# zoltanmaric/h264-fer

Measured on AMD Instinct MI355X. Metric: macroblocks/sec encode (1080p full-search ME) + bit-exact bitstream vs ref, higher is better.
Workload: dtype u8; 1 GPU; 1080p IPPP encode, full-search +-16 ME (BASELINE configs[2]); content=textured, coded_size=1920x1072, streams_per_gpu=256, contexts_per_gpu=1, gop=30, qp=12, window=32, maxdiff=3, parallelism=1 x 256 independent closed-GOP streams

## Files before the change

### h264-fer_amd/__init__.py

```python
from .ferhip import (FerHip, FerHipError, Decoder, LiveDecoder, access_units, DeviceBuffer, Y4MReader, decode_streams, unescape_nal, lib_path,
                     load_library, mb_unit, cavlc_blocks, mc_sub_mb_parts, MBU_QT, MBU_DEC4, MBU_DEC16, MBU_DECC, MBU_SKIP, TUNE_RESOLVE_WGS, TUNE_RESOLVE_GROUP, TUNE_SPECULATE, TUNE_OVERLAP_SORT, RC_CQP, RC_ABR, RC_QUALITY, QM_SSE, QM_SSIM,
                     QUALITY_RING, Quality, NAL_SLICE, NAL_IDR, NAL_AUTO, NAL_NONE, AU_PARAM_SETS, AU, frame_nal_blocks, frame_nal_blocks_raw,
                     NAL_UNIT, SPLIT_PREFIX, split_nal_blocks, split_nal_blocks_raw, FMT_I420, FMT_NV12, Pic, pic_table,
                     AU_AVCC, IN_ANNEXB, IN_AVCC, split_avcc_blocks_raw)
from .synth import gen_frame, gen_frames, crop_to_mb, pad_to_mb
from .shard import gops_of_rank, merge_gop_streams, split_nals
```

### h264-fer_amd/csrc/fer_internal.h

```cpp
#pragma once
#include "fer_dev.h"
#include "../../include/ferhip.h"

struct FerSortTmp {
    uint4 *rec1;
    uint16_t *keyT;
    uint8_t *dig2;
    uint16_t *skey;
    uint32_t *rec_tmp;
    void *tmp;
    size_t tmp_bytes;
};

size_t fer_sort_tmp_bytes(int n, int S);
void fer_launch_refprep(const FerDev &d, FerSortTmp &t, const int *types, hipStream_t st);
void fer_launch_interp(const FerDev &d, hipStream_t st);
void fer_launch_features(const FerDev &d, hipStream_t st);
void fer_launch_sort(const FerDev &d, FerSortTmp &t, hipStream_t st);
void fer_launch_sort_keys(const FerDev &d, FerSortTmp &t, hipStream_t st);
void fer_launch_sort_radix(const FerDev &d, FerSortTmp &t, hipStream_t st);
void fer_launch_sort_finish(const FerDev &d, FerSortTmp &t, hipStream_t st);
void fer_launch_me_walk(const FerDev &d, hipStream_t st);
void fer_launch_frame_sad(const FerDev &d, const uint8_t *skip, hipStream_t st);
void fer_launch_me_pre(const FerDev &d, hipStream_t st);
void fer_launch_me_spec(const FerDev &d, hipStream_t st);
void fer_launch_me_resolve(const FerDev &d, hipStream_t st);
void fer_launch_basic_stat(const FerDev &d, hipStream_t st);
void fer_launch_p_resid(const FerDev &d, hipStream_t st);
void fer_launch_intra(const FerDev &d, hipStream_t st);
void fer_launch_cavlc(const FerDev &d, hipStream_t st);
void fer_launch_rc_plan(const FerDev &d, hipStream_t st);
int fer_quality_groups(const FerDev &d);
void fer_launch_quality(const FerDev &d, int flags, int slot, hipStream_t st);
void fer_launch_carry_ref(const FerDev &d, hipStream_t st);
void fer_launch_reset_stream(const FerDev &d, int s, int qpw, hipStream_t st);
void fer_launch_decode_parse(const FerDev &d, const DecBatch &B, hipStream_t st);
void fer_launch_decode_recon(const FerDev &dslice, bool anyP, bool anyIntra, hipStream_t st);
void fer_launch_decode_out(const FerDev &d, const uint8_t *set, const int2 *map, int n, uint8_t *dst, hipStream_t st);
void fer_launch_decode_out_win(const FerDev &d, const uint8_t *set, const int2 *map, int n, uint8_t *dst, const int *win, hipStream_t st);
void fer_launch_pad_ingest(const FerDev &d, uint8_t *set, const uint8_t *src, int dw, int dh, const uint8_t *present, hipStream_t st);
void fer_launch_pic_ingest(const FerDev &d, uint8_t *set, const ferhip_pic *d_pics, int format, int dw, int dh, hipStream_t st);
void fer_launch_pic_emit(const FerDev &d, const uint8_t *set, const ferhip_pic *d_pics, int format, const int *win, hipStream_t st);
void fer_launch_pic_emit_slots(const FerDev &d, const uint8_t *set, const int2 *map, int n, uint8_t *dst, int format, uint32_t pitch_y,
                               uint32_t pitch_c, size_t slot_bytes, const int *win, hipStream_t st);
```

### h264-fer_amd/csrc/fer_mbunit.hip

```cpp
#include "fer_cavlc_dev.h"
#include "fer_ctx.h"

__device__ __forceinline__ void mbu_scan(const int c[16], int32_t *list, bool ac)
{
#pragma unroll
    for (int k = ac ? 1 : 0; k < 16; k++) list[ac ? k - 1 : k] = c[c_zz[k]];
    if (ac) list[15] = 0;
}
__device__ __forceinline__ void mbu_invscan(const int32_t *list, int c[16], bool ac, int dc)
{
#pragma unroll
    for (int k = 0; k < 16; k++) c[c_zz[k]] = ac ? (k == 0 ? dc : list[k - 1]) : list[k];
}

__global__ __launch_bounds__(64) void k_mb_unit(const ferhip_mb_job *jobs, ferhip_mb_result *res, int n)
{
    __shared__ int dcl[16], dcc[2][4], dcdeq[2][4], dcy[16];
    const int j = blockIdx.x, lane = threadIdx.x;
    if (j >= n) return;
    const ferhip_mb_job &J = jobs[j];
    ferhip_mb_result &R = res[j];
    const int op = J.op, qp = J.qp, qpc = J.qpc;
    const bool luma = lane < 16, chroma = lane >= 16 && lane < 24;
    const int blk = lane & 15, cpl = (lane - 16) >> 2, cblk = (lane - 16) & 3;
// ... 104 lines not shown
            int dq[16];
            mbu_invscan(J.dc16, cc, false, 0);
            inv_dc_luma(cc, dq, qp);
#pragma unroll
            for (int i = 0; i < 16; i++) dcy[i] = dq[i];
        }
        __syncthreads();
        if (luma) {
            mbu_invscan(J.ac16[blk], cc, true, dcy[(y0 >> 2) * 4 + (x0 >> 2)]);
            inv4x4(cc, r, qp, true);
            store_rec(r);
        }
    } else if (op == FERHIP_MBU_DECC) {
        if (lane == 16 || lane == 20) {
            int q[4], dq[4];
#pragma unroll
            for (int i = 0; i < 4; i++) q[i] = J.cdc[cpl][i];
            inv_dc_chroma(q, dq, qpc);
#pragma unroll
            for (int i = 0; i < 4; i++) dcdeq[cpl][i] = dq[i];
        }
        __syncthreads();
        if (chroma) {
            mbu_invscan(J.cac[cpl][cblk], cc, true, dcdeq[cpl][cblk]);
            inv4x4(cc, r, qpc, true);
            store_rec(r);
        }
    } else if (op == FERHIP_MBU_SKIP) {
#pragma unroll
        for (int i = 0; i < 16; i++) cc[i] = 0;
        inv4x4(cc, r, luma ? qp : qpc, !luma);
        if (luma || chroma) store_rec(r);
    }
}

extern "C" int ferhip_mb_unit(const ferhip_mb_job *jobs, ferhip_mb_result *results, size_t n)
{
    if (!jobs || !results || n == 0) return FERHIP_E_ARG;
    ferhip_mb_job *dj = nullptr;
    ferhip_mb_result *dr = nullptr;
    auto body = [&]() -> int {
        CK(hipMalloc((void **)&dj, n * sizeof *dj));
        CK(hipMalloc((void **)&dr, n * sizeof *dr));
        CK(hipMemcpy(dj, jobs, n * sizeof *dj, hipMemcpyHostToDevice));
        CK(hipMemset(dr, 0, n * sizeof *dr));
        hipLaunchKernelGGL(k_mb_unit, dim3((unsigned)n), dim3(64), 0, 0, dj, dr, (int)n);
        CK(hipGetLastError());
        CK(hipMemcpy(results, dr, n * sizeof *dr, hipMemcpyDeviceToHost));
        return 0;
    };
    const int rc = body();
    hipFree(dj);
    hipFree(dr);
    return rc;
}

__global__ __launch_bounds__(64) void k_cavlc_blocks(const int32_t *coef, const int32_t *nC, const int32_t *maxn, int n, uint32_t *bits,
                                                     uint32_t *nbits, int32_t *tc, uint32_t *nbits_size)
{
    __shared__ int16_t stage[16 * 64];
    const int i = blockIdx.x * 64 + threadIdx.x;
    if (i >= n) return;
    int16_t *st = stage + threadIdx.x;
    const int m = maxn[i];
    unsigned nz = 0;
#pragma unroll
    for (int k = 0; k < 16; k++) {
        const int v = k < m ? coef[(size_t)i * 16 + k] : 0;
        st[k * 64] = (int16_t)v;
        nz |= (v != 0 ? 1u : 0u) << k;
    }
    BitW w;
    bw_init<true>(w, bits + (size_t)i * 16, 16, 0);
    cavlc_block_core<true>(w, nz, m, nC[i], st, 64);
    bw_flush<true>(w);
    nbits[i] = w.bits;
    tc[i] = __popc(nz);
    BitW ws;
    bw_init<false>(ws, nullptr, 0, 0);
    cavlc_block_core<false>(ws, nz, m, nC[i], st, 64);
    nbits_size[i] = ws.bits;
}

extern "C" int ferhip_cavlc_blocks(const int32_t *coef, const int32_t *nC, const int32_t *max_num_coeff, size_t n, uint8_t *bits,
                                   uint32_t *nbits, int32_t *total_coeff)
{
    if (!coef || !nC || !max_num_coeff || !bits || !nbits || !total_coeff || n == 0) return FERHIP_E_ARG;
    int32_t *dc = nullptr, *dn = nullptr, *dm = nullptr, *dt = nullptr;
    uint32_t *db = nullptr, *dl = nullptr, *ds = nullptr;
    std::vector<uint32_t> sz(n);
    auto body = [&]() -> int {
        CK(hipMalloc((void **)&dc, n * 64));
        CK(hipMalloc((void **)&dn, n * 4));
        CK(hipMalloc((void **)&dm, n * 4));
        CK(hipMalloc((void **)&dt, n * 4));
        CK(hipMalloc((void **)&db, n * 64));
        CK(hipMalloc((void **)&dl, n * 4));
        CK(hipMalloc((void **)&ds, n * 4));
        CK(hipMemcpy(dc, coef, n * 64, hipMemcpyHostToDevice));
        CK(hipMemcpy(dn, nC, n * 4, hipMemcpyHostToDevice));
        CK(hipMemcpy(dm, max_num_coeff, n * 4, hipMemcpyHostToDevice));
        CK(hipMemset(db, 0, n * 64));
        hipLaunchKernelGGL(k_cavlc_blocks, dim3((unsigned)((n + 63) / 64)), dim3(64), 0, 0, dc, dn, dm, (int)n, db, dl, dt, ds);
        CK(hipGetLastError());
        CK(hipMemcpy(bits, db, n * 64, hipMemcpyDeviceToHost));
        CK(hipMemcpy(nbits, dl, n * 4, hipMemcpyDeviceToHost));
// ... 166 lines not shown
```

### h264-fer_amd/csrc/fer_me.hip

```cpp
#include <stdlib.h>
#include "fer_internal.h"
#include "fer_mvpred.h"

#define INF_M 1000000000

struct WList {
    int m;
    int xy;
};

__device__ __forceinline__ int pack_xy(int x, int y) { return (x & 0xffff) | (y << 16); }
__device__ __forceinline__ int unp_x(int xy) { return (int)(short)(xy & 0xffff); }
__device__ __forceinline__ int unp_y(int xy) { return xy >> 16; }

__device__ __forceinline__ void wl_insert(WList &L, int K, int lane, bool valid, int m, int xy)
{
    int thr = lane_bcast(L.m, K - 1);
    unsigned long long mask = __ballot(valid && m < thr);
    while (mask) {
        int src = __ffsll((long long)mask) - 1;
        mask &= mask - 1;
        int cm = lane_bcast(m, src), cxy = lane_bcast(xy, src);
        int pos = __popcll(__ballot(lane < K && L.m <= cm));
        if (pos < K) {
            int um = FER_DPP(L.m, DPP_WAVE_SHR1), uxy = FER_DPP(L.xy, DPP_WAVE_SHR1);
            if (lane > pos && lane < K) {
                L.m = um;
                L.xy = uxy;
            } else if (lane == pos) {
                L.m = cm;
                L.xy = cxy;
            }
        }
    }
}

#define WAVE_LDS_SYNC()                                    \
    do {                                                   \
        __builtin_amdgcn_fence(__ATOMIC_SEQ_CST, "wavefront"); \
        __builtin_amdgcn_wave_barrier();                   \
    } while (0)
__device__ __forceinline__ int lds_rank64(const unsigned *p, unsigned mine, int n4 = 16)
{
    const uint4 *q = (const uint4 *)p;
    int r = 0;
#pragma unroll 4
    for (int i = 0; i < n4; i++) {
        uint4 k = q[i];
        r += (int)(k.x < mine) + (int)(k.y < mine) + (int)(k.z < mine) + (int)(k.w < mine);
    }
    return r;
}

template <int NB, bool ORDERED, class RAW, class FIN, class ARR>
__device__ __forceinline__ bool select_topk_ex(const int (&v)[NB], int K, int lane, int *sel, WList &L, RAW raw, FIN fin, ARR arr)
{
    unsigned *A = (unsigned *)sel, *B = A + 64;
    int *Ci = sel + 128, *Di = sel + 192;
    const unsigned long long lt = (1ull << lane) - 1ull;
    int lmin = 0x7fffffff, lmax = -1, total = 0;
#pragma unroll
    for (int u = 0; u < NB; u++) {
        total += __popcll(__ballot(v[u] >= 0));
        lmin = (int)min((unsigned)lmin, (unsigned)v[u]);
        lmax = max(lmax, v[u]);
    }
    const int need = min(K, total);
    L.m = INF_M;
    L.xy = 0;
    if (need == 0) return true;
    int c = 65;
    if (!__any(lmax >= (1 << 26))) {
        B[lane] = 0xffffffffu;
        int T0 = 0x7fffffff;
        if (__popcll(__ballot(lmin != 0x7fffffff)) >= need) {
            int lo = 0, hi = (1 << 21) - 1;
            if (__popcll(__ballot(lmin <= hi)) >= need) {
                while (lo < hi) {
                    const int mid = (lo + hi) >> 1;
                    if (__popcll(__ballot(lmin <= mid)) >= need)
                        hi = mid;
                    else
                        lo = mid + 1;
                }
                T0 = lo;
            } else {
                T0 = 1 << 21;
            }
        }
        WAVE_LDS_SYNC();
        if (T0 < (1 << 21) && NB * 64 <= 2048) {
            int nsurv = 0;
#pragma unroll
            for (int u = 0; u < NB; u++) {
                const bool take = (unsigned)v[u] <= (unsigned)T0;
                const unsigned long long mk = __ballot(take);
                if (mk) {
                    const int slot = nsurv + (int)__builtin_amdgcn_mbcnt_hi((uint32_t)(mk >> 32), __builtin_amdgcn_mbcnt_lo((uint32_t)mk, 0u));
                    if (take && slot < 64) {
                        B[slot] = ((unsigned)v[u] << 11) | (unsigned)arr(u);
                        Ci[slot] = raw(u);
                    }
                    nsurv += __popcll(mk);
                }
            }
            WAVE_LDS_SYNC();
            c = nsurv;
        }
    }
    if (c <= 64) {
        WAVE_LDS_SYNC();
        const unsigned mine = B[lane];
        const int mypay = Ci[lane];
        const int rk = lds_rank64(B, mine, (__builtin_amdgcn_readfirstlane(c) + 3) >> 2);
        WAVE_LDS_SYNC();
        if (lane < c && rk < need) {
            A[rk] = mine >> 11;
            Di[rk] = mypay;
        }
        WAVE_LDS_SYNC();
        if (lane < need) {
            L.m = (int)A[lane];
            L.xy = fin(Di[lane]);
        }
        WAVE_LDS_SYNC();
        return true;
    }
    if (!ORDERED) return false;
    int *key = sel, *kxy = sel + 64, *key2 = sel + 128, *kxy2 = sel + 192;
    int lo = wave_min(lmin), hi;
    if (__popcll(__ballot(lmin != 0x7fffffff)) >= need)
        hi = wave_max(lmin != 0x7fffffff ? lmin : -1);
    else
        hi = wave_max(lmax);
    while (lo < hi) {
        int mid = lo + ((hi - lo) >> 1);
        int cnt = 0;
#pragma unroll
        for (int u = 0; u < NB; u++) cnt += __popcll(__ballot(v[u] >= 0 && v[u] <= mid));
        if (cnt >= need)
            hi = mid;
        else
// ... 332 lines not shown
    su[4] = wave_sum((px & 3) > 1 ? 0 : v);
    if (lane < 5) d.suma[pidx * 5 + lane] = su[lane];
    if (d.basic) {
        if (lane == 0) {
            d.st3n[pidx] = 0;
            d.v0[pidx] = 0;
        }
        return;
    }
    const SuPk sp = su_pack(su);
    PP_MARK(0)

    WList L;
    L.m = INF_M;
    L.xy = 0;
    const int R = window / 2, n = 2 * R + 1;
    const int r2 = window / 16, n2w = 2 * r2 + 1, nloc = n2w * n2w * 16;
    const uint16_t *F0 = d.feat0 + (size_t)s * 6 * ysz;
    const int wb = (n * n + 63) >> 6;
    if ((WIN == 32 || WIN == 16) && !FER_DBGF(d, 3)) {
        constexpr int WCH = 6;
        constexpr int NN = (WIN ? WIN : 32) + 1;
        constexpr int NBc = WIN ? WIN : 32, RPB = 64 / NBc, NWB = (NN + RPB - 1) / RPB;
        constexpr int LB = LocalGeo<RRL>::NB;
        static_assert(LB <= 7, "ME_SEL_NB leaves room for 7 local batches");
        const int ix = lane % NBc, r0 = lane / NBc;
        const int rx = sx - R + ix;
        const bool xok = rx >= 0 && rx < W;
        const int wx = iabs(ix - R) + 4;
        const uint32_t colo = (uint32_t)iclamp(rx, 0, W - 1) * 12u, rowb = (uint32_t)W * 12u;
        auto fin = [&](int idx) {
            if (idx < wb * 64) return pack_xy((idx / n - R) * 4, (idx % n - R) * 4);
            int c = idx - wb * 64;
            int frac = c & 15, pos = c >> 4;
            return pack_xy((pos / n2w - r2) * 4 + (frac & 3), (pos % n2w - r2) * 4 + (frac >> 2));
        };
        uint32_t k0w[NWB];
#pragma unroll
        for (int b2 = 0; b2 < NWB; b2++) {
            const int ry = iclamp(sy - R + b2 * RPB + r0, 0, H - 1);
            k0w[b2] = *(const uint32_t *)((const char *)F0 + (colo + __umul24((uint32_t)ry, rowb)));
        }
        const uint32_t k0c = feat0_load(F0, W, H, sy - R + min(lane, NN - 1), sx + R).a;
        local_metrics<RRL>(ip, W, H, sx - r2, sy - r2, sp, lane, (uint32_t *)wide_m, sel_lds, 0, 2, &ld);
        int vloc[LB];
        unsigned lminl = 0xffffffffu;
#pragma unroll
        for (int u = 0; u < LB; u++) {
            vloc[u] = sel_lds[u * 64 + lane];
            lminl = min(lminl, (unsigned)vloc[u]);
        }
        int T = 0x7fffffff;
        if (__popcll(__ballot(lminl < (1u << 21))) >= 33) {
            int lo = 0, hi = (1 << 21) - 1;
            while (lo < hi) {
                const int mid = (lo + hi) >> 1;
                if (__popcll(__ballot(lminl <= (unsigned)mid)) >= 33)
                    hi = mid;
                else
                    lo = mid + 1;
            }
            T = lo;
        }
        int *surv = wide_m;
        int ns = 0;
        const uint32_t s0 = (uint32_t)su[0];
        bool done = false;
        if (T != 0x7fffffff) {
#pragma unroll
            for (int b2 = 0; b2 < NWB; b2++) {
                const int iy = b2 * RPB + r0;
                const int ry = sy - R + iy;
                const uint32_t lb = __umul24(5u * (uint32_t)(wx + iabs(iy - R)), __builtin_amdgcn_sad_u16(k0w[b2] & 0xffffu, s0, 0u));
                const bool take = xok && ry >= 0 && ry < H && iy < NN && lb <= (uint32_t)T;
                const unsigned long long mk = __ballot(take);
                if (mk) {
                    const int slot = ns + (int)__builtin_amdgcn_mbcnt_hi((uint32_t)(mk >> 32), __builtin_amdgcn_mbcnt_lo((uint32_t)mk, 0u));
                    if (take && slot < 128) surv[slot] = ix * NN + iy;
                    ns += __popcll(mk);
                }
            }
            {
                const int iy = lane, ry = sy - R + iy;
                const uint32_t lb = __umul24(5u * (uint32_t)(R + 4 + iabs(iy - R)), __builtin_amdgcn_sad_u16(k0c & 0xffffu, s0, 0u));
                const bool take = iy < NN && sx + R < W && ry >= 0 && ry < H && lb <= (uint32_t)T;
                const unsigned long long mk = __ballot(take);
                if (mk) {
                    const int slot = ns + (int)__builtin_amdgcn_mbcnt_hi((uint32_t)(mk >> 32), __builtin_amdgcn_mbcnt_lo((uint32_t)mk, 0u));
                    if (take && slot < 128) surv[slot] = (NN - 1) * NN + iy;
                    ns += __popcll(mk);
                }
            }
            WAVE_LDS_SYNC();
            if (ns <= 128) {
                int v[2 + LB], ar[2];
#pragma unroll
                for (int b2 = 0; b2 < 2; b2++) {
                    v[b2] = -1;
                    ar[b2] = 0;
                    if (b2 * 64 < ns) {
                        const int idx = b2 * 64 + lane;
                        const bool on = idx < ns;
                        const int ai = on ? surv[idx] : 0;
                        const int cix = ai / NN, ciy = ai - cix * NN;
                        const FeatRec f = feat0_load(F0, W, H, sy - R + ciy, sx - R + cix);
                        const int m = (int)__umul24((uint32_t)(iabs(cix - R) + iabs(ciy - R) + 4), (uint32_t)feat_dist_w(f.a, f.b, f.c, sp));
                        v[b2] = on ? m : -1;
                        ar[b2] = ai;
                    }
                }
#pragma unroll
                for (int u = 0; u < LB; u++) v[2 + u] = vloc[u];
                WAVE_LDS_SYNC();
                auto arrv = [&](int u) { return u < 2 ? ar[u < 2 ? u : 0] : wb * 64 + (u - 2) * 64 + lane; };
                done = select_topk_ex<2 + LB, false>(v, 33, lane, sel_lds, L, arrv, fin, arrv);
            }
        }
        PP_MARK(1)
#ifdef FER_STATS
        if (lane == 0) {
            atomicAdd((unsigned long long *)&d.timing[48], 1ull);
            atomicAdd((unsigned long long *)&d.timing[49], done ? 0ull : 1ull);
            atomicAdd((unsigned long long *)&d.timing[50], (unsigned long long)ns);
            atomicAdd((unsigned long long *)&d.timing[51], T == 0x7fffffff ? 1ull : 0ull);
            atomicAdd((unsigned long long *)&d.timing[52], (unsigned long long)(T == 0x7fffffff ? 0 : T));
        }
#endif
        if (!done) {
            WAVE_LDS_SYNC();
            auto wide_load = [&](int iy0, FeatRec (&fr)[WCH]) {
#pragma unroll
                for (int q = 0; q < WCH; q++) {
                    int ry = iclamp(sy - R + iy0 + q * RPB + r0, 0, H - 1);
                    const uint32_t *r = (const uint32_t *)((const char *)F0 + (colo + __umul24((uint32_t)ry, rowb)));
                    fr[q].a = r[0];
                    fr[q].b = r[1];
                    fr[q].c = r[2];
                }
            };
            auto wide_eval = [&](int iy0, const FeatRec (&fr)[WCH]) {
#pragma unroll
                for (int q = 0; q < WCH; q++) {
                    const int iy = iy0 + q * RPB + r0;
                    const int ry = sy - R + iy;
                    const int m = (int)__umul24((uint32_t)(wx + iabs(iy - R)), (uint32_t)feat_dist_w(fr[q].a, fr[q].b, fr[q].c, sp));
                    const int bad = (xok && ry >= 0 && ry < H) ? 0 : -1;
                    wide_m[iy < n ? ix * n + iy : ME_WIDE_LDS - 1] = m | bad;
                }
            };
            {
                constexpr int STEP = RPB * WCH;
                FeatRec fa[WCH], fb[WCH];
                wide_load(0, fa);
                for (int iy0 = 0; iy0 < n; iy0 += 2 * STEP) {
                    if (iy0 + STEP < n) wide_load(iy0 + STEP, fb);
                    wide_eval(iy0, fa);
                    if (iy0 + STEP < n) {
                        if (iy0 + 2 * STEP < n) wide_load(iy0 + 2 * STEP, fa);
                        wide_eval(iy0 + STEP, fb);
                    }
                }
            }
            {
                const int iy = min(lane, n - 1);
                const int rxl = sx + R, ry = sy - R + iy;
                FeatRec f = feat0_load(F0, W, H, ry, rxl);
                int m = (R + 4 + iabs(iy - R)) * feat_dist_w(f.a, f.b, f.c, sp);
                if (!(rxl < W && ry >= 0 && ry < H)) m = -1;
                if (lane < n) wide_m[(n - 1) * n + iy] = m;
            }
            __syncthreads();
            int v[ME_SEL_NB];
#pragma unroll
            for (int u = 0; u < ME_SEL_NB; u++) {
                v[u] = -1;
                if (u < wb) {
                    int c = u * 64 + lane;
                    if (c < n * n) v[u] = wide_m[c];
                } else if (u - wb < LB) {
                    v[u] = vloc[u - wb < LB ? u - wb : 0];
                }
            }
            WAVE_LDS_SYNC();
            auto raw = [&](int u) { return u * 64 + lane; };
            PP_MARK(2)
            select_topk<ME_SEL_NB>(v, 33, lane, sel_lds, L, raw, fin);
        }
        PP_MARK(3)
    } else {
        for (int base = 0; base < n * n && !FER_DBGF(d, 1); base += 64) {
            int c = base + lane;
            int tx = c / n - R, ty = c % n - R;
            int rx = sx + tx, ry = sy + ty;
            bool ok = c < n * n && rx >= 0 && rx < W && ry >= 0 && ry < H;
            int m = 0;
            if (ok) m = (iabs(tx) + iabs(ty) + 4) * feat_dist_rec(F0 + ((size_t)ry * W + rx) * 6, sp);
            wl_insert(L, 33, lane, ok, m, pack_xy(tx * 4, ty * 4));
        }
        for (int base = 0; base < nloc && !FER_DBGF(d, 2); base += 64) {
            int c = base + lane;
            int frac = c & 15, pos = c >> 4;
            int tx = pos / n2w - r2, ty = pos % n2w - r2;
            int rx = sx + tx, ry = sy + ty;
            bool ok = c < nloc && rx >= 0 && rx < W && ry >= 0 && ry < H;
            int m = 0;
            if (ok) {
                const FeatRec f = feat_rec_direct(ip, W, H, frac, ry, rx);
                m = (iabs(tx) + iabs(ty) + 4) * feat_dist_w(f.a, f.b, f.c, sp);
            }
            wl_insert(L, 33, lane, ok, m, pack_xy(tx * 4 + (frac & 3), ty * 4 + (frac >> 2)));
        }
    }
    const int n3 = __popcll(__ballot(lane < 33 && L.m < 100000000));
    int v0 = 0;
    if (!FER_DBGF(d, 4)) {
        const SrcBlk SB = src_block_load(Y, W, sx, sy);
        const int cx = unp_x(L.xy), cy = unp_y(L.xy);
        const int sad = sad_lane(ip, W, H, sx, sy, lane < n3 ? cx : 0, lane < n3 ? cy : 0, SB);
        if (lane < n3) {
            int *o = d.st3 + (pidx * 33 + lane) * 3;
            o[0] = cx;
            o[1] = cy;
            o[2] = sad;
        }
        const int wk = wave_min(lane < n3 ? (sad << 6) | lane : 0x7fffffff);
        if (wk != 0x7fffffff) v0 = lane_bcast(L.xy, wk & 63);
    }
    if (lane == 0) {
        d.st3n[pidx] = n3;
        d.v0[pidx] = v0;
    }

}

__device__ __forceinline__ bool wave_mask_bit(unsigned long long m) { return __builtin_amdgcn_inverse_ballot_w64(m); }
__device__ __forceinline__ unsigned long long wave_ballot(bool p) { return __builtin_amdgcn_ballot_w64(p); }
struct NoProbe {
    __device__ __forceinline__ int operator()(int) const { return 0; }
};
template <bool QUIRK, class SINK, class PROBE = NoProbe>
__device__ __forceinline__ int walk_buckets_q(const FerDev &d, int s, const int (&su)[5], const SuPk &sp, int sx, int sy, int lane,
                                              uint32_t *tbl, int halt_cnt, int &jend, SINK sink, uint32_t max_slice = 0xffffffffu,
                                              bool skip0 = false, PROBE probe = PROBE())
{
    int tren = 0;
    jend = 180;
    const int kt = d.kt;
    const uint32_t *kol2 = d.kol2 + (size_t)s * 16384 * kt;
    const uint32_t *srec = d.sort_rec;
    const int n0 = QUIRK ? d.zero_cnt[s] : 0;
    const uint32_t npos = (uint32_t)(d.W * d.H), g0 = (uint32_t)s * npos;
    const uint16_t *F0 = d.feat0 + (size_t)s * 6 * d.ysz;
    const int t_lo = QUIRK ? 0 : (max(sx - 279, 0) >> d.ktw_shift), t_hi = QUIRK ? kt - 1 : (min(sx + 279, d.W - 1) >> d.ktw_shift);
    auto qstart = [&](int a) -> uint32_t {
        if (a <= 0) return g0;
        if (a == 1) return g0 + min(2u * (uint32_t)n0, npos);
        if (a >= 16384) return g0 + npos;
        return kol2[(size_t)a * kt] - (uint32_t)n0;
    };
    const uint32_t sxy = ((uint32_t)sx << 16) | (uint32_t)sy;
    const char *srec_s = (const char *)(srec + (size_t)g0 * 3);
    auto fetch = [&](unsigned b_start, int b_cnt, uint32_t &r0, uint32_t &r1, uint32_t &r2) {
        const uint32_t li = (b_start - g0) + (unsigned)min(lane, max(b_cnt - 1, 0));
        const uint32_t *e = (const uint32_t *)(srec_s + __umul24(li, 12u));
        r0 = e[0];
        r1 = e[1];
        r2 = e[2];
    };
    auto passes = [&](uint32_t r0, uint32_t r1) -> bool {
        uint32_t dist = __builtin_amdgcn_sad_u16(r0, sxy, 0);
        uint32_t e12 = pk_abs16(pk_sub16(r1, sp.s12));
        return dist < 280u && (pk_sub16(e12, 0x00640064u) & 0x80008000u) == 0x80008000u;
    };
    auto passes_mask = [&](uint32_t r0, uint32_t r1) -> unsigned long long {
        uint32_t dist = __builtin_amdgcn_sad_u16(r0, sxy, 0);
        uint32_t e12 = pk_abs16(pk_sub16(r1, sp.s12));
        return wave_ballot(dist < 280u) & wave_ballot((pk_sub16(e12, 0x00640064u) & 0x80008000u) == 0x80008000u);
    };
    auto feat_d = [&](uint32_t info, uint32_t r0, uint32_t r1, uint32_t r2) -> uint32_t {
        uint32_t D;
        if (!QUIRK) {
            const uint32_t aa = ((info >> 16) & 0x7fffu) * 0x10001u;
            D = __builtin_amdgcn_sad_u16(r1, sp.s12, (info >> 8) & 255u);
            D = __builtin_amdgcn_sad_u16(r2, sp.s34, D);
            D = __builtin_amdgcn_sad_u16(pk_sub16(aa, r1), sp.e12, D);
            D = __builtin_amdgcn_sad_u16(pk_sub16(aa, r2), sp.e34, D);
        } else {
            int px = min((int)(r0 >> 16), d.W - 1), py = min((int)(r0 & 0xffff), d.H - 1);
            D = (uint32_t)feat_dist_rec(F0 + ((size_t)py * d.W + px) * 6, sp);
// ... 1102 lines not shown
        d.timing[7] = gw;
    }
#undef PR_MARK
    if (timeout && lane == 0) atomicOr(&d.status[s], FER_ERR_CHAIN_TIMEOUT);
    }
    if (lane == 0 && st_parts + st_skq > 0) {
        atomicAdd(&d.spec_stat[0], (unsigned long long)st_parts);
        atomicAdd(&d.spec_stat[1], (unsigned long long)st_hits);
        atomicAdd(&d.spec_stat[2], (unsigned long long)st_skq);
        atomicAdd(&d.spec_stat[3], (unsigned long long)st_skh);
    }
}

__global__ __launch_bounds__(64) void k_basic_stat(FerDev d)
{
    const int lane = threadIdx.x;
    const int s = blockIdx.y, mb = blockIdx.x;
    if (d.hdr[s * 4 + 3] != 0) return;
    if (d.mb_type[(size_t)s * d.nmb + mb] == FER_P_SKIP) return;
    const int W = d.W, H = d.H;
    const uint8_t *Y = d.curY + (size_t)s * d.ysz;
    const uint8_t *RY = d.refY + (size_t)s * d.ysz;
    const IPlanes ip = ip_stream(d, s);
    const int xp = (mb % d.mbw) << 4, yp = (mb / d.mbw) << 4;
    int src[4][4];
#pragma unroll
    for (int y = 0; y < 4; y++) {
        uint32_t v = *(const uint32_t *)(Y + (size_t)(yp + y) * W + xp);
#pragma unroll
        for (int k = 0; k < 4; k++) src[y][k] = (v >> (8 * k)) & 0xff;
    }
    const int R = d.window / 2, n = 2 * R + 1;
    int bsad = 0x7fffffff, bidx = 0x7fffffff;
    for (int c = lane; c < n * n; c += 64) {
        const int mvx = c / n - R, mvy = c % n - R;
        int sad = 0;
#pragma unroll
        for (int y = 0; y < 4; y++) {
            int p[4];
            mc_luma4(RY, ip, W, H, xp, yp, 0, y, mvx, mvy, p);
#pragma unroll
            for (int k = 0; k < 4; k++) sad += iabs(src[y][k] - p[k]);
        }
        if (sad < bsad) {
            bsad = sad;
            bidx = c;
        }
    }
    const int wsad = wave_min(bsad);
    const int widx = wave_min(bsad == wsad ? bidx : 0x7fffffff);
    if (lane == 0) atomicAdd(&d.stats[s * 5 + (widx == 0 ? 1 : 4)], 1);
}

void fer_launch_basic_stat(const FerDev &d, hipStream_t st)
{
    if (d.basic) hipLaunchKernelGGL(k_basic_stat, dim3(d.nmb, d.S), dim3(64), 0, st, d);
}

void fer_launch_me_pre(const FerDev &d, hipStream_t st)
{
    dim3 g(d.nmb * 4, d.S);
    if (d.window == 32)
        hipLaunchKernelGGL(k_me_pre<32>, g, dim3(64), 0, st, d);
    else if (d.window == 16)
        hipLaunchKernelGGL(k_me_pre<16>, g, dim3(64), 0, st, d);
    else
        hipLaunchKernelGGL(k_me_pre<0>, g, dim3(64), 0, st, d);
}

void fer_launch_me_walk(const FerDev &d, hipStream_t st)
{
    if (d.basic) return;
    hipLaunchKernelGGL(k_me_walk, dim3(d.nmb * 4, d.S), dim3(64), 0, st, d);
}

void fer_launch_me_spec(const FerDev &d, hipStream_t st)
{
    if (!d.speculate) return;
    dim3 g(d.nmb, d.S);
    if (d.window == 32)
        hipLaunchKernelGGL(k_me_spec<32>, g, dim3(256), 0, st, d);
    else if (d.window == 16)
        hipLaunchKernelGGL(k_me_spec<16>, g, dim3(256), 0, st, d);
    else
        hipLaunchKernelGGL(k_me_spec<0>, g, dim3(256), 0, st, d);
}

void fer_launch_me_resolve(const FerDev &d, hipStream_t st)
{
    const int gh = 2 * d.mbh;
    hipMemsetAsync(d.chain, 0, sizeof(int) * 8, st);
    const int cap = d.resolve_wgs;
    dim3 g(min(gh * d.S, max(cap, 1)));
    if (d.window == 32)
        hipLaunchKernelGGL(k_me_resolve<32>, g, dim3(64), 0, st, d);
    else if (d.window == 16)
        hipLaunchKernelGGL(k_me_resolve<16>, g, dim3(64), 0, st, d);
    else
        hipLaunchKernelGGL(k_me_resolve<0>, g, dim3(64), 0, st, d);
}
```

### h264-fer_amd/ferhip.py

```python
import ctypes as C
import math
import os
from pathlib import Path

import numpy as np

NAL_SLICE, NAL_IDR, NAL_AUTO = 1, 5, 0
NAL_NONE = -1

BUF = dict(INTERP=1, FEAT=2, SORTPOS=3, KOLIKO=4, MBTYPE=5, MV=6, MVD=7, LEVELS=8, CBP=9, TC=10, I4MODE=11,
           CUR=12, REF=13, TIMING=14, ST2N=15, ST2=16, SPEC_STAT=17, MBSIZE=18,
           SUMA=19, ST3=20, ST3N=21, V0=22, SPEC_HDR=23, SPEC_L1=24, SPEC_L2=25)
TUNE_RESOLVE_WGS, TUNE_RESOLVE_GROUP, TUNE_SPECULATE, TUNE_OVERLAP_SORT = 1, 2, 3, 4
RC_CQP, RC_ABR, RC_QUALITY = 0, 1, 2
QM_SSE, QM_SSIM, QUALITY_RING = 1, 2, 64
AU_PARAM_SETS = 1
AU_AVCC = 4
IN_ANNEXB, IN_AVCC = 0, 1
_BUF_DTYPE = {1: np.uint8, 2: np.uint16, 3: np.uint32, 4: np.int32, 5: np.int32, 6: np.int16, 7: np.int16,
              8: np.int16, 9: np.uint8, 10: np.uint8, 11: np.uint8, 12: np.uint8, 13: np.uint8, 14: np.int64, 15: np.int32, 16: np.int32,
              17: np.uint64, 18: np.int32, 19: np.int32, 20: np.int32, 21: np.int32, 22: np.int32, 23: np.int32, 24: np.int32,
              25: np.int32}


# ... 498 lines not shown
        return list(a)


def forward_residual(qp, blocks, keep_dc=False):
    lib = load_library()
    a = np.ascontiguousarray(blocks, np.int32).reshape(-1, 16)
    out = np.empty_like(a)
    _chk(lib.ferhip_forward_residual(qp, a.ctypes.data, out.ctypes.data, int(keep_dc), a.shape[0]),
         "ferhip_forward_residual")
    return out


def inverse_residual(qp, blocks, keep_dc=False):
    lib = load_library()
    a = np.ascontiguousarray(blocks, np.int32).reshape(-1, 16)
    out = np.empty_like(a)
    _chk(lib.ferhip_inverse_residual(qp, a.ctypes.data, out.ctypes.data, int(keep_dc), a.shape[0]),
         "ferhip_inverse_residual")
    return out


class MbJob(C.Structure):
    _fields_ = [("op", C.c_int32), ("cls", C.c_int32), ("qp", C.c_int32), ("qpc", C.c_int32), ("reconstruct", C.c_int32), ("blk", C.c_int32),
                ("srcY", C.c_int32 * 256), ("srcCb", C.c_int32 * 64), ("srcCr", C.c_int32 * 64),
                ("predY", C.c_int32 * 256), ("predCb", C.c_int32 * 64), ("predCr", C.c_int32 * 64),
                ("lumaLevel", C.c_int32 * 256), ("dc16", C.c_int32 * 16), ("ac16", C.c_int32 * 256), ("cdc", C.c_int32 * 8), ("cac", C.c_int32 * 128)]


class MbResult(C.Structure):
    _fields_ = [("lumaLevel", C.c_int32 * 256), ("dc16", C.c_int32 * 16), ("ac16", C.c_int32 * 256), ("cdc", C.c_int32 * 8), ("cac", C.c_int32 * 128),
                ("recY", C.c_int32 * 256), ("recCb", C.c_int32 * 64), ("recCr", C.c_int32 * 64)]


MBU_QT, MBU_DEC4, MBU_DEC16, MBU_DECC, MBU_SKIP = range(5)


def mb_unit(jobs):
    lib = load_library()
    n = len(jobs)
    J = (MbJob * n)()
    R = (MbResult * n)()
    for k, j in enumerate(jobs):
        for name, val in j.items():
            if isinstance(val, (int, np.integer)):
                setattr(J[k], name, int(val))
            else:
                a = np.ascontiguousarray(val, np.int32).reshape(-1)
                C.memmove(getattr(J[k], name), a.ctypes.data, a.nbytes)
    lib.ferhip_mb_unit.argtypes = [C.c_void_p, C.c_void_p, C.c_size_t]
    _chk(lib.ferhip_mb_unit(J, R, n), "ferhip_mb_unit")
    return [{f: np.frombuffer(getattr(R[k], f), np.int32).copy() for f, _ in MbResult._fields_} for k in range(n)]


def cavlc_blocks(coef, nC, max_num_coeff):
    lib = load_library()
    c = np.ascontiguousarray(coef, np.int32).reshape(-1, 16)
    n = c.shape[0]
    nc = np.ascontiguousarray(nC, np.int32)
    mx = np.ascontiguousarray(max_num_coeff, np.int32)
    bits = np.zeros((n, 64), np.uint8)
    nb = np.zeros(n, np.uint32)
    tc = np.zeros(n, np.int32)
    lib.ferhip_cavlc_blocks.argtypes = [C.c_void_p] * 3 + [C.c_size_t] + [C.c_void_p] * 3
    _chk(lib.ferhip_cavlc_blocks(c.ctypes.data, nc.ctypes.data, mx.ctypes.data, n, bits.ctypes.data, nb.ctypes.data, tc.ctypes.data), "ferhip_cavlc_blocks")
    return bits, nb, tc


def frame_nal_blocks_raw(payloads, nal_types, cap=None, fill=0xA5, flags=None):
    lib = load_library()
    n = len(payloads)
    lens = np.array([len(p) for p in payloads], np.uint32)
    stride = max(int(lens.max()) if n else 0, 1)
    src = np.zeros((n, stride), np.uint8)
    for k, p in enumerate(payloads):
        src[k, : len(p)] = np.frombuffer(bytes(p), np.uint8) if not isinstance(p, np.ndarray) else p
    if cap is None:
        cap = int(sum(((int(m) * 3 // 2 + 6 + 15) & ~15) for m in lens))
    out = np.full(max(int(cap), 1), fill, np.uint8)
    idx = np.zeros(n + 1, AU)
    nt = np.ascontiguousarray(nal_types, np.int32)
    if flags is None:
        rc = lib.ferhip_frame_nal_blocks(src.ctypes.data, stride, lens.ctypes.data, nt.ctypes.data, n, out.ctypes.data, int(cap),
                                         idx.ctypes.data)
    else:
        rc = lib.ferhip_frame_nal_blocks_fmt(src.ctypes.data, stride, lens.ctypes.data, nt.ctypes.data, n, int(flags), out.ctypes.data,
                                             int(cap), idx.ctypes.data)
    return rc, out, idx


def split_nal_blocks_raw(ranges, misalign=0, cap=None, units_cap=None, fill=0xA5):
    lib = load_library()
    n = len(ranges)
    lens = np.array([len(r) for r in ranges], np.uint32)
    stride = max(int(lens.max()) if n else 0, 1)
    src = np.zeros((n, stride), np.uint8)
    for k, r in enumerate(ranges):
        src[k, : len(r)] = np.frombuffer(bytes(r), np.uint8) if not isinstance(r, np.ndarray) else r
    if cap is None:
        cap = int(sum((int(m) // 5 + 1) * 16 + int(m) for m in lens))
    if units_cap is None:
        units_cap = int(sum(int(m) // 5 + 1 for m in lens))
    out = np.full(max(int(cap), 1), fill, np.uint8)
    units = np.zeros(max(int(units_cap), 1), NAL_UNIT)
    count = C.c_size_t(0)
    rc = lib.ferhip_split_nal_blocks(src.ctypes.data, stride, lens.ctypes.data, n, int(misalign), out.ctypes.data, int(cap),
                                     units.ctypes.data, int(units_cap), C.byref(count))
# ... 309 lines not shown
```

### include/ferhip.h

```cpp
#ifndef FERHIP_H
#define FERHIP_H
#include <stddef.h>
#include <stdint.h>

#ifdef __cplusplus
extern "C" {
#endif

#define FERHIP_E_ARG -1
#define FERHIP_E_HIP -2
#define FERHIP_E_STATE -3
#define FERHIP_E_UNSUP -4
#define FERHIP_E_DEVICE -5

#define FERHIP_NAL_SLICE 1
#define FERHIP_NAL_IDR 5
#define FERHIP_NAL_AUTO 0
#define FERHIP_NAL_NONE -1

typedef struct ferhip_ctx ferhip_ctx;

typedef struct {
    int qp;
    int basic;
// ... 171 lines not shown

#define FERHIP_SPLIT_PREFIX 64
typedef struct { uint32_t range; int32_t nal_type, ref_idc; uint32_t bytes; uint64_t offset; } ferhip_nal_unit;
int ferhip_split_nal_blocks(const uint8_t *ranges, size_t stride, const uint32_t *lens, size_t n, int misalign, uint8_t *out,
                            size_t cap, ferhip_nal_unit *units, size_t units_cap, size_t *nunits);
int ferhip_decs_decode_dev(ferhip_decs *d, const uint8_t *const *d_chunks, const size_t *lens, uint8_t *out, int out_on_device,
                           int *pictures, int *status);
int ferhip_decs_timing(ferhip_decs *d, double *t , int reset);

#define FERHIP_IN_ANNEXB 0
#define FERHIP_IN_AVCC 1
int ferhip_decs_set_input(ferhip_decs *d, int format, int length_size);
int ferhip_decs_set_config(ferhip_decs *d, int s, const uint8_t *avcc, size_t n);
int ferhip_split_avcc_blocks(const uint8_t *ranges, size_t stride, const uint32_t *lens, size_t n, int misalign, int length_size,
                             uint8_t *out, size_t cap, ferhip_nal_unit *units, size_t units_cap, size_t *nunits,
                             int32_t *range_fault );

typedef struct ferhip_y4m ferhip_y4m;
int ferhip_y4m_open(ferhip_y4m **out, const char *path, int *in_width, int *in_height, int *coded_width, int *coded_height);
int ferhip_y4m_read(ferhip_y4m *y, unsigned char *dst);
void ferhip_y4m_close(ferhip_y4m *y);
int ferhip_y4m_write_header(void *file, int width, int height);
int ferhip_y4m_write_frame(void *file, const unsigned char *i420, int width, int height, int with_frame_line);

int ferhip_forward_residual(int qP, const int32_t *in, int32_t *out, int keep_dc, size_t nblocks);
int ferhip_inverse_residual(int qP, const int32_t *in, int32_t *out, int keep_dc, size_t nblocks);
int ferhip_forward_dc_luma_intra(int qP, const int32_t *in, int32_t *out, size_t nblocks);
int ferhip_inverse_dc_luma_intra(int qP, const int32_t *in, int32_t *out, size_t nblocks);
int ferhip_forward_dc_chroma(int qP, const int32_t *in, int32_t *out, size_t nblocks);
int ferhip_inverse_dc_chroma(int qP, const int32_t *in, int32_t *out, size_t nblocks);
int ferhip_transform_scan(const int32_t *in, int32_t *out, int intra16x16_ac, size_t nblocks);
int ferhip_transform_inverse_scan(const int32_t *in, int32_t *out, size_t nblocks);

#define FERHIP_MBU_QT 0
#define FERHIP_MBU_DEC4 1
#define FERHIP_MBU_DEC16 2
#define FERHIP_MBU_DECC 3
#define FERHIP_MBU_SKIP 4
typedef struct {
    int32_t op, cls , qp , qpc , reconstruct, blk;
    int32_t srcY[256], srcCb[64], srcCr[64];
    int32_t predY[256], predCb[64], predCr[64];
    int32_t lumaLevel[16][16], dc16[16], ac16[16][16], cdc[2][4], cac[2][4][16];
} ferhip_mb_job;
typedef struct {
    int32_t lumaLevel[16][16], dc16[16], ac16[16][16], cdc[2][4], cac[2][4][16];
    int32_t recY[256], recCb[64], recCr[64];
} ferhip_mb_result;
int ferhip_mb_unit(const ferhip_mb_job *jobs, ferhip_mb_result *results, size_t njobs);
int ferhip_cavlc_blocks(const int32_t *coef, const int32_t *nC, const int32_t *max_num_coeff, size_t nblocks, uint8_t *bits,
                        uint32_t *nbits, int32_t *total_coeff);
int ferhip_mc_sub_mb_parts(const uint8_t *ref_i420, int width, int height, const int32_t *desc, size_t n, int32_t *predL,
                           int32_t *predCb, int32_t *predCr);

#ifdef __cplusplus
}
#endif
#endif
```

Measured before the change: 22.23 million macroblocks/s.

## Replace ME top-k binary search with bitwise kth-min and reuse known threshold

Replaces the ballot-driven binary search for the K-th smallest lane minimum in the ME top-k selection with a fixed bit-by-bit radix descent. Blocks of high bits are skipped when a bound is known. When the survivor scan already yields the exact threshold, that value is reused directly. The LDS rank count uses inline asm compare-with-carry adds, and the local candidate values are spilled to LDS in the wide fallback path to cut register pressure. A host test entry point for the selection routine is also added, which does not affect the encode path.

```diff
diff --git a/h264-fer_amd/__init__.py b/h264-fer_amd/__init__.py
--- a/h264-fer_amd/__init__.py
+++ b/h264-fer_amd/__init__.py
@@ -2,6 +2,6 @@
                      load_library, mb_unit, cavlc_blocks, mc_sub_mb_parts, MBU_QT, MBU_DEC4, MBU_DEC16, MBU_DECC, MBU_SKIP, TUNE_RESOLVE_WGS, TUNE_RESOLVE_GROUP, TUNE_SPECULATE, TUNE_OVERLAP_SORT, RC_CQP, RC_ABR, RC_QUALITY, QM_SSE, QM_SSIM,
                      QUALITY_RING, Quality, NAL_SLICE, NAL_IDR, NAL_AUTO, NAL_NONE, AU_PARAM_SETS, AU, frame_nal_blocks, frame_nal_blocks_raw,
                      NAL_UNIT, SPLIT_PREFIX, split_nal_blocks, split_nal_blocks_raw, FMT_I420, FMT_NV12, Pic, pic_table,
-                     AU_AVCC, IN_ANNEXB, IN_AVCC, split_avcc_blocks_raw)
+                     AU_AVCC, IN_ANNEXB, IN_AVCC, split_avcc_blocks_raw, select_kat)
 from .synth import gen_frame, gen_frames, crop_to_mb, pad_to_mb
 from .shard import gops_of_rank, merge_gop_streams, split_nals
diff --git a/h264-fer_amd/csrc/fer_internal.h b/h264-fer_amd/csrc/fer_internal.h
--- a/h264-fer_amd/csrc/fer_internal.h
+++ b/h264-fer_amd/csrc/fer_internal.h
@@ -25,6 +25,8 @@
 void fer_launch_me_pre(const FerDev &d, hipStream_t st);
 void fer_launch_me_spec(const FerDev &d, hipStream_t st);
 void fer_launch_me_resolve(const FerDev &d, hipStream_t st);
+bool fer_launch_select_kat(int nb, int k, int ordered, const int32_t *metric, const int32_t *arrival, const int32_t *bound, int32_t *out,
+                           unsigned ncases);
 void fer_launch_basic_stat(const FerDev &d, hipStream_t st);
 void fer_launch_p_resid(const FerDev &d, hipStream_t st);
 void fer_launch_intra(const FerDev &d, hipStream_t st);
diff --git a/h264-fer_amd/csrc/fer_mbunit.hip b/h264-fer_amd/csrc/fer_mbunit.hip
--- a/h264-fer_amd/csrc/fer_mbunit.hip
+++ b/h264-fer_amd/csrc/fer_mbunit.hip
@@ -180,6 +180,45 @@
     const int rc = body();
     hipFree(dj);
     hipFree(dr);
+    return rc;
+}
+
+extern "C" int ferhip_select_kat(int nb, int k, int ordered, const int32_t *metric, const int32_t *arrival, const int32_t *bound, size_t n,
+                                 int32_t *out)
+{
+    if (!metric || !out || n == 0 || n > (1u << 20) || nb < 1 || nb > 32) return FERHIP_E_ARG;
+    if (ordered ? (arrival || bound) : !arrival) return FERHIP_E_ARG;
+    const size_t per = (size_t)nb * 64;
+    for (size_t i = 0; i < n * per; i++) {
+        if (metric[i] < -1 || metric[i] > (1 << 28)) return FERHIP_E_ARG;
+        if (!ordered && (arrival[i] < 0 || arrival[i] >= 2048)) return FERHIP_E_ARG;
+    }
+    for (size_t i = 0; bound && i < n; i++)
+        if (bound[i * 2] >= (1 << 21)) return FERHIP_E_ARG;
+    int32_t *dm = nullptr, *da = nullptr, *db = nullptr, *dout = nullptr;
+    auto body = [&]() -> int {
+        CK(hipMalloc((void **)&dm, n * per * 4));
+        CK(hipMemcpy(dm, metric, n * per * 4, hipMemcpyHostToDevice));
+        if (arrival) {
+            CK(hipMalloc((void **)&da, n * per * 4));
+            CK(hipMemcpy(da, arrival, n * per * 4, hipMemcpyHostToDevice));
+        }
+        if (bound) {
+            CK(hipMalloc((void **)&db, n * 2 * 4));
+            CK(hipMemcpy(db, bound, n * 2 * 4, hipMemcpyHostToDevice));
+        }
+        CK(hipMalloc((void **)&dout, n * FERHIP_SELECT_KAT_OUT * 4));
+        CK(hipMemset(dout, 0, n * FERHIP_SELECT_KAT_OUT * 4));
+        if (!fer_launch_select_kat(nb, k, ordered, dm, da, db, dout, (unsigned)n)) return FERHIP_E_ARG;
+        CK(hipGetLastError());
+        CK(hipMemcpy(out, dout, n * FERHIP_SELECT_KAT_OUT * 4, hipMemcpyDeviceToHost));
+        return 0;
+    };
+    const int rc = body();
+    hipFree(dm);
+    hipFree(da);
+    hipFree(db);
+    hipFree(dout);
     return rc;
 }
 
diff --git a/h264-fer_amd/csrc/fer_me.hip b/h264-fer_amd/csrc/fer_me.hip
--- a/h264-fer_amd/csrc/fer_me.hip
+++ b/h264-fer_amd/csrc/fer_me.hip
@@ -35,25 +35,68 @@
     }
 }
 
+__device__ __forceinline__ bool wave_mask_bit(unsigned long long m) { return __builtin_amdgcn_inverse_ballot_w64(m); }
+__device__ __forceinline__ unsigned long long wave_ballot(bool p) { return __builtin_amdgcn_ballot_w64(p); }
+
 #define WAVE_LDS_SYNC()                                    \
     do {                                                   \
         __builtin_amdgcn_fence(__ATOMIC_SEQ_CST, "wavefront"); \
         __builtin_amdgcn_wave_barrier();                   \
     } while (0)
+__device__ __forceinline__ int rank_add4(int r, uint4 k, unsigned mine)
+{
+    unsigned long long m0, m1, m2, m3;
+    asm("v_cmp_lt_u32_e64 %1, %5, %9\n\t"
+        "v_cmp_lt_u32_e64 %2, %6, %9\n\t"
+        "v_cmp_lt_u32_e64 %3, %7, %9\n\t"
+        "v_cmp_lt_u32_e64 %4, %8, %9\n\t"
+        "v_addc_co_u32_e64 %0, %1, 0, %0, %1\n\t"
+        "v_addc_co_u32_e64 %0, %2, 0, %0, %2\n\t"
+        "v_addc_co_u32_e64 %0, %3, 0, %0, %3\n\t"
+        "v_addc_co_u32_e64 %0, %4, 0, %0, %4"
+        : "+v"(r), "=&s"(m0), "=&s"(m1), "=&s"(m2), "=&s"(m3)
+        : "v"(k.x), "v"(k.y), "v"(k.z), "v"(k.w), "v"(mine));
+    return r;
+}
 __device__ __forceinline__ int lds_rank64(const unsigned *p, unsigned mine, int n4 = 16)
 {
     const uint4 *q = (const uint4 *)p;
     int r = 0;
 #pragma unroll 4
-    for (int i = 0; i < n4; i++) {
-        uint4 k = q[i];
-        r += (int)(k.x < mine) + (int)(k.y < mine) + (int)(k.z < mine) + (int)(k.w < mine);
-    }
+    for (int i = 0; i < n4; i++) r = rank_add4(r, q[i], mine);
     return r;
 }
 
-template <int NB, bool ORDERED, class RAW, class FIN, class ARR>
-__device__ __forceinline__ bool select_topk_ex(const int (&v)[NB], int K, int lane, int *sel, WList &L, RAW raw, FIN fin, ARR arr)
+template <bool BOUNDED = false>
+__device__ __forceinline__ int lane_kth_min21(unsigned lmin, int need, int bound = (1 << 21) - 1)
+{
+    int T = 0;
+    asm("" : "+s"(need));
+    auto step = [&](int b) {
+        const int t = T | (1 << b);
+        const int cnt = __builtin_popcountll(wave_ballot(lmin < (unsigned)t));
+        T = cnt < need ? t : T;
+    };
+    if (!BOUNDED || bound >= (1 << 17)) {
+#pragma unroll
+        for (int b = 20; b >= 17; b--) step(b);
+    }
+    if (!BOUNDED || bound >= (1 << 13)) {
+#pragma unroll
+        for (int b = 16; b >= 13; b--) step(b);
+    }
+    if (!BOUNDED || bound >= (1 << 9)) {
+#pragma unroll
+        for (int b = 12; b >= 9; b--) step(b);
+    }
+#pragma unroll
+    for (int b = 8; b >= 0; b--) step(b);
+    return T;
+}
+
+template <int NB, bool ORDERED, bool BOUNDED = false, class RAW, class FIN, class ARR>
+__device__ __forceinline__ bool select_topk_ex(const int (&v)[NB], int K, int lane, int *sel, WList &L, RAW raw, FIN fin, ARR arr,
+                                               int bound = (1 << 21) - 1, bool bound_exact = false, int *t0_out = nullptr)
 {
     unsigned *A = (unsigned *)sel, *B = A + 64;
     int *Ci = sel + 128, *Di = sel + 192;
@@ -74,20 +117,16 @@
         B[lane] = 0xffffffffu;
         int T0 = 0x7fffffff;
         if (__popcll(__ballot(lmin != 0x7fffffff)) >= need) {
-            int lo = 0, hi = (1 << 21) - 1;
-            if (__popcll(__ballot(lmin <= hi)) >= need) {
-                while (lo < hi) {
-                    const int mid = (lo + hi) >> 1;
-                    if (__popcll(__ballot(lmin <= mid)) >= need)
-                        hi = mid;
-                    else
-                        lo = mid + 1;
-                }
-                T0 = lo;
+            if (__popcll(__ballot(lmin <= (1 << 21) - 1)) >= need) {
+                if (BOUNDED && bound_exact)
+                    T0 = bound;
+                else
+                    T0 = lane_kth_min21<BOUNDED>((unsigned)lmin, need, bound);
             } else {
                 T0 = 1 << 21;
             }
         }
+        if (t0_out) *t0_out = T0;
         WAVE_LDS_SYNC();
         if (T0 < (1 << 21) && NB * 64 <= 2048) {
             int nsurv = 0;
@@ -526,15 +565,7 @@
         }
         int T = 0x7fffffff;
         if (__popcll(__ballot(lminl < (1u << 21))) >= 33) {
-            int lo = 0, hi = (1 << 21) - 1;
-            while (lo < hi) {
-                const int mid = (lo + hi) >> 1;
-                if (__popcll(__ballot(lminl <= (unsigned)mid)) >= 33)
-                    hi = mid;
-                else
-                    lo = mid + 1;
-            }
-            T = lo;
+            T = lane_kth_min21(lminl, 33);
         }
         int *surv = wide_m;
         int ns = 0;
@@ -587,7 +618,7 @@
                 for (int u = 0; u < LB; u++) v[2 + u] = vloc[u];
                 WAVE_LDS_SYNC();
                 auto arrv = [&](int u) { return u < 2 ? ar[u < 2 ? u : 0] : wb * 64 + (u - 2) * 64 + lane; };
-                done = select_topk_ex<2 + LB, false>(v, 33, lane, sel_lds, L, arrv, fin, arrv);
+                done = select_topk_ex<2 + LB, false, true>(v, 33, lane, sel_lds, L, arrv, fin, arrv, T, ns == 0);
             }
         }
         PP_MARK(1)
@@ -602,6 +633,8 @@
 #endif
         if (!done) {
             WAVE_LDS_SYNC();
+#pragma unroll
+            for (int u = 0; u < LB; u++) sel_lds[u * 64 + lane] = vloc[u];
             auto wide_load = [&](int iy0, FeatRec (&fr)[WCH]) {
 #pragma unroll
                 for (int q = 0; q < WCH; q++) {
@@ -652,7 +685,7 @@
                     int c = u * 64 + lane;
                     if (c < n * n) v[u] = wide_m[c];
                 } else if (u - wb < LB) {
-                    v[u] = vloc[u - wb < LB ? u - wb : 0];
+                    v[u] = sel_lds[(u - wb < LB ? u - wb : 0) * 64 + lane];
                 }
             }
             WAVE_LDS_SYNC();
@@ -707,8 +740,6 @@
 
 }
 
-__device__ __forceinline__ bool wave_mask_bit(unsigned long long m) { return __builtin_amdgcn_inverse_ballot_w64(m); }
-__device__ __forceinline__ unsigned long long wave_ballot(bool p) { return __builtin_amdgcn_ballot_w64(p); }
 struct NoProbe {
     __device__ __forceinline__ int operator()(int) const { return 0; }
 };
@@ -1917,6 +1948,59 @@
     if (lane == 0) atomicAdd(&d.stats[s * 5 + (widx == 0 ? 1 : 4)], 1);
 }
 
+template <int NB, int K, bool ORDERED>
+__global__ __launch_bounds__(64) void k_select_kat(const int32_t *metric, const int32_t *arrival, const int32_t *bound, int32_t *out)
+{
+    __shared__ __attribute__((aligned(16))) int sel_lds[256];
+    const int lane = threadIdx.x;
+    const size_t c = blockIdx.x;
+    int v[NB], ar[NB];
+#pragma unroll
+    for (int u = 0; u < NB; u++) {
+        v[u] = metric[(c * NB + u) * 64 + lane];
+        ar[u] = ORDERED ? u * 64 + lane : arrival[(c * NB + u) * 64 + lane];
+    }
+    WList L;
+    int t0 = -1;
+    auto tag = [&](int u) { return ar[u]; };
+    auto fin = [&](int t) { return t; };
+    bool done;
+    const int bnd = bound ? bound[c * 2] : -1;
+    if constexpr (!ORDERED) {
+        if (bnd >= 0)
+            done = select_topk_ex<NB, false, true>(v, K, lane, sel_lds, L, tag, fin, tag, bnd, bound[c * 2 + 1] != 0, &t0);
+        else
+            done = select_topk_ex<NB, false>(v, K, lane, sel_lds, L, tag, fin, tag, (1 << 21) - 1, false, &t0);
+    } else {
+        done = select_topk_ex<NB, true>(v, K, lane, sel_lds, L, tag, fin, tag, (1 << 21) - 1, false, &t0);
+    }
+    int32_t *o = out + c * FERHIP_SELECT_KAT_OUT;
+    if (lane == 0) {
+        o[0] = t0;
+        o[1] = done ? 0 : 1;
+    }
+    o[2 + lane] = L.m;
+    o[66 + lane] = L.xy;
+}
+
+bool fer_launch_select_kat(int nb, int k, int ordered, const int32_t *metric, const int32_t *arrival, const int32_t *bound, int32_t *out,
+                           unsigned ncases)
+{
+#define SELECT_KAT_FORM(NB_, K_, ORD_)                                                                                      \
+    if (nb == NB_ && k == K_ && (ordered != 0) == ORD_) {                                                                   \
+        hipLaunchKernelGGL((k_select_kat<NB_, K_, ORD_>), dim3(ncases), dim3(64), 0, 0, metric, arrival, bound, out);       \
+        return true;                                                                                                        \
+    }
+    SELECT_KAT_FORM(7, 17, true)
+    SELECT_KAT_FORM(3, 17, true)
+    SELECT_KAT_FORM(6, 33, true)
+    SELECT_KAT_FORM(9, 33, false)
+    SELECT_KAT_FORM(5, 33, false)
+    SELECT_KAT_FORM(25, 33, true)
+#undef SELECT_KAT_FORM
+    return false;
+}
+
 void fer_launch_basic_stat(const FerDev &d, hipStream_t st)
 {
     if (d.basic) hipLaunchKernelGGL(k_basic_stat, dim3(d.nmb, d.S), dim3(64), 0, st, d);
diff --git a/h264-fer_amd/ferhip.py b/h264-fer_amd/ferhip.py
--- a/h264-fer_amd/ferhip.py
+++ b/h264-fer_amd/ferhip.py
@@ -574,6 +574,25 @@
     return [{f: np.frombuffer(getattr(R[k], f), np.int32).copy() for f, _ in MbResult._fields_} for k in range(n)]
 
 
+SELECT_KAT_OUT = 130
+
+
+def select_kat(metric, k, arrival=None, bound=None):
+    lib = load_library()
+    m = np.ascontiguousarray(metric, np.int32)
+    n, nb, lanes = m.shape
+    assert lanes == 64
+    a = None if arrival is None else np.ascontiguousarray(arrival, np.int32)
+    b = None if bound is None else np.ascontiguousarray(bound, np.int32)
+    assert a is None or a.shape == m.shape
+    assert b is None or b.shape == (n, 2)
+    out = np.zeros((n, SELECT_KAT_OUT), np.int32)
+    lib.ferhip_select_kat.argtypes = [C.c_int] * 3 + [C.c_void_p] * 3 + [C.c_size_t, C.c_void_p]
+    _chk(lib.ferhip_select_kat(nb, int(k), int(a is None), m.ctypes.data, None if a is None else a.ctypes.data,
+                               None if b is None else b.ctypes.data, n, out.ctypes.data), "ferhip_select_kat")
+    return {"threshold": out[:, 0].copy(), "refused": out[:, 1] != 0, "metric": out[:, 2:66].copy(), "tag": out[:, 66:130].copy()}
+
+
 def cavlc_blocks(coef, nC, max_num_coeff):
     lib = load_library()
     c = np.ascontiguousarray(coef, np.int32).reshape(-1, 16)
diff --git a/include/ferhip.h b/include/ferhip.h
--- a/include/ferhip.h
+++ b/include/ferhip.h
@@ -247,6 +247,9 @@
                         uint32_t *nbits, int32_t *total_coeff);
 int ferhip_mc_sub_mb_parts(const uint8_t *ref_i420, int width, int height, const int32_t *desc, size_t n, int32_t *predL,
                            int32_t *predCb, int32_t *predCr);
+#define FERHIP_SELECT_KAT_OUT 130
+int ferhip_select_kat(int nb, int k, int ordered, const int32_t *metric, const int32_t *arrival, const int32_t *bound, size_t ncases,
+                      int32_t *out);
 
 #ifdef __cplusplus
 }
```

After: 22.15 million macroblocks/s. About the same (-0.3%).
